# Farama-Foundation/Gymnasium-Robotics

Hardware: NVIDIA H100
Metric: env-steps/s (higher is better)
Workload: dtype f32

## Files before the change

### gymnasium_robotics_b200/csrc/b200sim.cu

```cuda
#include <cuda_runtime.h>
#include <stdio.h>
#include <stdlib.h>
#include <string>
#include <vector>

#include "../../include/b200sim.h"
#include "step_kernel.cuh"
#include "reset_sample.cuh"

#define B200_WPB_MAX 32

#ifdef B200_STAGE_TIMING
extern "C" int b200sim_debug_stage_cycles(unsigned long long* out, int reset) {
  cudaDeviceSynchronize();
  cudaMemcpyFromSymbol(out, g_stage_cycles, sizeof(unsigned long long) * TM_COUNT);
  if (reset) { unsigned long long z[TM_COUNT] = {0}; cudaMemcpyToSymbol(g_stage_cycles, z, sizeof(z)); }
  return TM_COUNT;
}
#endif

__global__ void reward_kernel(const float* __restrict__ ag, const float* __restrict__ dg, int M, int ngoal, int kind, float thr,
                              float radius, int dense, FetchTask task, float* __restrict__ out) {
  int i = blockIdx.x * blockDim.x + threadIdx.x;
  if (i >= M) return;
// ... 201 lines not shown
  if (t.kind == TASK_FETCH) { t.nact = 4; t.ngoal = 3; }
  if (t.kind == TASK_ADROIT_HAMMER) {
    bool ok = t.nact == dh->nu && t.ngoal == 3 && t.nobs == dh->nq - 6 + 6 + 13 && dh->nsensor <= 1 && t.penv_body > 0 && t.penv_body < dh->nb;
    const int sites[5] = {t.grip_site, t.obj_site, t.frame_site, t.tip_site[0], t.tip_site[1]};
    for (int k = 0; k < 5; k++) ok = ok && sites[k] >= 0 && sites[k] < dh->nsite;
    if (!ok) { delete h; return fail(nullptr, "b200sim_create: inconsistent AdroitHandHammer task", -6); }
  }
  if (t.kind == TASK_ADROIT_DOOR) {
    bool ok = t.nact == dh->nu && t.ngoal == 3 && t.nobs == dh->nq - 3 + 12 && t.penv_body > 0 && t.penv_body < dh->nb &&
              t.obj_qadr >= 0 && t.obj_qadr < dh->nq && t.grip_site >= 0 && t.grip_site < dh->nsite && t.frame_site >= 0 && t.frame_site < dh->nsite;
    if (!ok) { delete h; return fail(nullptr, "b200sim_create: inconsistent AdroitHandDoor task", -6); }
  }
  if (t.kind == TASK_ADROIT_PEN) {
    bool ok = t.nact == dh->nu && t.ngoal == 3 && t.nobs == dh->nq - 6 + 21 && t.penv_body > 0 && t.penv_body < dh->nb &&
              t.distance_threshold > 0 && t.rotation_threshold > 0;
    const int sites[6] = {t.obj_site, t.frame_site, t.tip_site[0], t.tip_site[1], t.tip_site[2], t.tip_site[3]};
    for (int k = 0; k < 6; k++) ok = ok && sites[k] >= 0 && sites[k] < dh->nsite;
    if (!ok) { delete h; return fail(nullptr, "b200sim_create: inconsistent AdroitHandPen task", -6); }
  }
  if (t.kind == TASK_ADROIT_RELOCATE) {
    bool ok = t.nact == dh->nu && t.ngoal == 3 && t.nobs == dh->nq - 6 + 9 && t.penv_body > 0 && t.penv_body < dh->nb &&
              t.grip_site >= 0 && t.grip_site < dh->nsite && t.obj_site >= 0 && t.obj_site < dh->nsite;
    if (!ok) { delete h; return fail(nullptr, "b200sim_create: inconsistent AdroitHandRelocate task", -6); }
  }
  if (t.kind == TASK_KITCHEN) {
    if (!(h->kitchen && t.nact == dh->nu && t.ngoal == dh->nq && t.nobs == dh->nq + dh->nv)) { delete h; return fail(nullptr, "b200sim_create: inconsistent FrankaKitchen task", -6); }
  } else if (h->kitchen) { delete h; return fail(nullptr, "b200sim_create: this model needs the kitchen task kind (8)", -6); }
  if (t.kind != TASK_FETCH && t.kind != TASK_ANTMAZE && t.kind != TASK_HAND && t.kind != TASK_HAND_REACH && !TASK_IS_ADROIT(t.kind) && t.kind != TASK_KITCHEN) { delete h; return fail(nullptr, "b200sim_create: unknown task kind", -6); }
  if (t.kind == TASK_HAND && (t.nact != dh->nu || t.ngoal != 7 || t.obj_qadr != dh->nq - 7 || t.obj_dadr != dh->nv - 6 ||
                              t.touch_mode < 0 || t.touch_mode > 3 || (t.touch_mode && dh->nsensor == 0) ||
                              t.nobs != t.obj_qadr + dh->nv + 7 + (t.touch_mode ? dh->nsensor : 0))) { delete h; return fail(nullptr, "b200sim_create: inconsistent Hand task", -6); }
  if (t.kind == TASK_FETCH && dh->nmocap != 1) { delete h; return fail(nullptr, "b200sim_create: Fetch task needs exactly one mocap body", -6); }
  if (t.kind == TASK_ANTMAZE && (t.nact != dh->nu || t.ngoal != 2 || t.touch_mode < 0 || t.touch_mode > 1 ||
                                 t.nobs != dh->nq - t.obs_qpos_start + dh->nv + (t.touch_mode == 1 ? 6 * (dh->nmjb - 1) : 0))) { delete h; return fail(nullptr, "b200sim_create: inconsistent AntMaze task", -6); }
  if (t.kind == TASK_HAND_REACH) {
    bool ok = t.nact == dh->nu && t.ngoal == 15 && t.nobs == dh->nq + dh->nv + 15;
    for (int k = 0; k < 5; k++) ok = ok && t.tip_site[k] >= 0 && t.tip_site[k] < dh->nsite;
    if (!ok) { delete h; return fail(nullptr, "b200sim_create: inconsistent HandReach task", -6); }
  }
  int o = 0;
  t.st_qpos = o; o += dh->nq; t.st_qvel = o; o += dh->nv; t.st_warm = o; o += dh->nv; t.st_ctrl = o; o += dh->nu;
  t.st_mocap = o; o += 7 * dh->nmocap; t.st_pose = o; o += (t.kind == TASK_FETCH ? 7 : 0); t.st_goal = o; o += t.ngoal;
  t.st_penv = o; o += (t.penv_body > 0 ? 7 : 0);
  t.st_stride = (o + 3) & ~3;
  DevGuard guard(device);
  if (!guard.ok) { delete h; return fail(nullptr, "b200sim_create: cudaSetDevice failed", -7); }
  int nsm = 132;
  cudaDeviceGetAttribute(&nsm, cudaDevAttrMultiProcessorCount, device);
  h->nvp = dh->nv <= 14 ? 14 : (dh->nv == 15 ? 15 : (dh->nv <= 21 ? 21 : (dh->nv <= 30 ? 30 : (dh->nv > 32 && dh->nv <= B200_WIDE_NVP ? B200_WIDE_NVP : 0))));
  if (h->nvp == 0) { delete h; return fail(nullptr, "b200sim_create: no kernel instantiation for this nv (31, 32 or > 36)", -8); }
  if ((t.kind == TASK_HAND || t.kind == TASK_HAND_REACH || TASK_IS_ADROIT(t.kind)) && h->nvp < 30) h->nvp = 30;
  if (dh->nv <= 21 && dh->any_convex_pair) h->nvp = 22;
  if (dh->nv <= 21 && (dh->nten > 0 || dh->nfric > 0 || dh->nsensor > 0 || dh->any_round_pair)) h->nvp = 30;
  auto fits = [&](int w) { return ((size_t)dh->hot_words + (size_t)w * dh->scr_words) * 4 + 64 <= 232448; };
  auto built = [&](int w) {
    if (h->nvp == B200_WIDE_NVP) return w == 7 || w == 10 || w == 13 || w == 14;
    bool b = false;
#define B200_HAS(W, V) b = b || (w == W && h->nvp == V);
    B200_FOR_ALL_VARIANTS(B200_HAS)
#undef B200_HAS
    return b;
  };
  const char* ov = getenv("B200SIM_WPB");
  const int ovw = ov ? atoi(ov) : 0;
  if (h->kitchen) {
    if (dh->nv > 31) { delete h; return fail(nullptr, "b200sim_create: the kitchen build is instantiated for nv <= 31", -8); }
    h->nvp = B200_KITCHEN_NVP;
    h->wpb = (num_envs + nsm - 1) / nsm <= 7 ? 7 : ((h->kitchen_groups && fits(11)) ? 11 : (fits(10) ? 10 : 7));
    if (ov) {
      if (!((ovw == 7 || ovw == 10 || (ovw == 11 && h->kitchen_groups)) && fits(ovw))) { delete h; return fail(nullptr, "b200sim_create: B200SIM_WPB names no kitchen kernel variant that fits", -8); }
      h->wpb = ovw;
    }
  } else {
    auto waves = [&](int w) { return ((num_envs + w - 1) / w + nsm - 1) / nsm; };
    int wmax = 0;
    for (int w = 1; w <= B200_WPB_MAX; w++)
      if (built(w) && fits(w)) wmax = w;
    h->wpb = wmax > 0 ? wmax : 7;
    for (int w = wmax; w >= 1; w--)
      if (built(w) && fits(w) && waves(w) == waves(wmax)) h->wpb = w;
    if (ov) {
      if (!(built(ovw) && fits(ovw))) { delete h; return fail(nullptr, "b200sim_create: B200SIM_WPB names no kernel variant that fits", -8); }
      h->wpb = ovw;
    }
  }
  if (!fits(h->wpb)) { delete h; return fail(nullptr, "b200sim_create: the per-env scratch of this model does not fit the shared memory of one block", -8); }
  h->smem_bytes = ((size_t)dh->hot_words + (size_t)h->wpb * dh->scr_words) * 4;
  h->blocks = (num_envs + h->wpb - 1) / h->wpb;
  h->packed_w = (t.nobs + 2 * t.ngoal + 4 + 3) & ~3;
  cudaError_t e = cudaErrorInvalidValue;
#define B200_SETATTR(W, V) if (h->wpb == W && h->nvp == V) e = cudaFuncSetAttribute(fetch_kernel<W, V>, cudaFuncAttributeMaxDynamicSharedMemorySize, (int)h->smem_bytes);
  B200_FOR_ALL_VARIANTS(B200_SETATTR)
#undef B200_SETATTR
  if (h->nvp == B200_WIDE_NVP) e = b200sim_wide_setattr(h->wpb, (int)h->smem_bytes) == 0 ? cudaSuccess : cudaErrorInvalidValue;
  if (h->nvp == B200_KITCHEN_NVP) e = (h->hull ? b200sim_kitchen_hull_setattr(h->wpb, (int)h->smem_bytes) : (h->kitchen_groups ? b200sim_kitchen_groups_setattr(h->wpb, (int)h->smem_bytes) : b200sim_kitchen_setattr(h->wpb, (int)h->smem_bytes))) == 0 ? cudaSuccess : cudaErrorInvalidValue;
  if (e != cudaSuccess) { std::string m = std::string("b200sim_create: no kernel variant <") + std::to_string(h->wpb) + ", " + std::to_string(h->nvp) + "> or cudaFuncSetAttribute(smem=" + std::to_string(h->smem_bytes) + ") failed: " + cudaGetErrorString(e); delete h; return fail(nullptr, m, -8); }
  const size_t state_bytes = (size_t)num_envs * t.st_stride * 4;
  if (cudaMalloc(&h->model_dev, h->model_host.size() * 4) != cudaSuccess || cudaMalloc(&h->state, state_bytes) != cudaSuccess ||
      cudaMalloc(&h->elapsed, (size_t)num_envs * 4) != cudaSuccess || cudaMalloc(&h->overflow_count, 8) != cudaSuccess) {
    free_handle(h); return fail(nullptr, "b200sim_create: cudaMalloc failed", -9);
  }
  if (cudaMemcpy(h->model_dev, h->model_host.data(), h->model_host.size() * 4, cudaMemcpyHostToDevice) != cudaSuccess ||
      cudaMemset(h->state, 0, state_bytes) != cudaSuccess || cudaMemset(h->elapsed, 0, (size_t)num_envs * 4) != cudaSuccess ||
      cudaMemset(h->overflow_count, 0, 8) != cudaSuccess) {
    free_handle(h); return fail(nullptr, "b200sim_create: uploading the model / clearing the state failed", -9);
  }
// ... 215 lines not shown
```

### gymnasium_robotics_b200/csrc/dmodel.h

```cpp
#pragma once
#include <stdint.h>
#include <string.h>
#include <math.h>
#include <vector>
#include <string>
#include <map>
#include <set>
#include <utility>

#include "../../include/b200sim_model.h"

#define DM_MAX_BODY 32
#define DM_MAX_NV 40
#define DM_NDOFROW_MIN 8
#define DM_NCAND_MAX 96
#define DM_NWELD_MAX 1
#define DM_CSLOT_WORDS 40

#ifdef B200_KITCHEN_GROUPS
#define DM_PAIR_HOT(X)
#define DM_PAIR_COLD(X) X(pair_geom1, 1, npair) X(pair_geom2, 1, npair) X(pair_margin, 1, npair)
#define DM_BGRP_HOT(X) X(bg_body, 1, nbgrp) X(bg_anchor, 1, nbgrp) X(bg_start, 1, nbgrp) X(bg_count, 1, nbgrp) X(bg_center, 3, nbgrp) X(bg_radius, 1, nbgrp)
#ifndef DM_NSURV_MAX
#define DM_NSURV_MAX 96
#endif
#else
#define DM_PAIR_HOT(X) X(pair_geom1, 1, npair) X(pair_geom2, 1, npair) X(pair_margin, 1, npair)
#define DM_PAIR_COLD(X)
#define DM_BGRP_HOT(X)
#endif
#ifdef B200_HULL
#define DM_HULL_COLD(X) X(geom_hull, 2, ngeom) X(hull_vert, 3, nhullv)
#else
#define DM_HULL_COLD(X)
#endif
#define DM_ARRAYS_HOT(X) \
  X(body_parent, 1, nb) X(body_jntadr, 1, nb) X(body_jntnum, 1, nb) X(body_dofadr, 1, nb) X(body_dofnum, 1, nb) \
  X(body_mocapid, 1, nb) X(body_ancdof, MW, nb) X(body_sub, 1, nb) X(body_pos, 3, nb) X(body_quat, 4, nb) \
  X(body_ipos, 3, nb) X(body_iquat, 4, nb) X(body_mass, 1, nb) X(body_inertia, 3, nb) \
  X(jnt_type, 1, njnt) X(jnt_body, 1, njnt) X(jnt_qposadr, 1, njnt) X(jnt_dofadr, 1, njnt) X(jnt_limited, 1, njnt) \
  X(jnt_pos, 3, njnt) X(jnt_axis, 3, njnt) X(jnt_range, 2, njnt) X(jnt_margin, 1, njnt) X(jnt_stiffness, 1, njnt) \
  X(jnt_qpos0, 1, njnt) X(jnt_qspring, 1, njnt) \
  X(dof_body, 1, nv) X(dof_jnt, 1, nv) X(dof_anc, MW, nv) X(dof_pre, MW, nv) X(dof_armature, 1, nv) \
  X(dof_damping, 1, nv) X(dof_frictionloss, 1, nv) X(dof_invweight0, 1, nv) \
  X(geom_type, 1, ngeom) X(geom_body, 1, ngeom) X(geom_pos, 3, ngeom) X(geom_quat, 4, ngeom) X(geom_size, 3, ngeom) \
  X(geom_rbound, 1, ngeom) \
  DM_PAIR_HOT(X) DM_BGRP_HOT(X) \
  X(site_body, 1, nsite) X(site_pos, 3, nsite) X(site_quat, 4, nsite) \
  X(act_trnid, 1, nu) X(act_ctrllimited, 1, nu) X(act_forcelimited, 1, nu) X(act_gear, 1, nu) X(act_gain, 1, nu) \
  X(act_bias, 3, nu) X(act_ctrlrange, 2, nu) X(act_forcerange, 2, nu) \
  X(eq_type, 1, neq) X(eq_obj1, 1, neq) X(eq_obj2, 1, neq) X(eq_active, 1, neq) X(eq_data, 11, neq) X(eq_solref, 2, neq) \
  X(eq_solimp, 5, neq) X(eq_invweight, 2, neq) \
  X(mocap_body, 1, nmocap) X(grid_walls, 1, ngridw) \
  X(dof_fricD, 1, nfric) X(dof_fricB, 1, nfric) \
  X(ten_dof, 2, nten) X(ten_qadr, 2, nten) X(ten_coef, 2, nten) X(ten_range, 2, nten) X(ten_margin, 1, nten)
#define DM_ARRAYS_COLD(X) \
  X(jnt_solref, 2, njnt) X(jnt_solimp, 5, njnt)  \
  DM_PAIR_COLD(X) \
  X(pair_condim, 1, npair) X(pair_friction, 3, npair) X(pair_gap, 1, npair) X(pair_solref, 2, npair) \
  X(pair_solimp, 5, npair) X(pair_invweight, 2, npair) \
  X(ten_solref, 2, nten) X(ten_solimp, 5, nten) X(ten_invweight, 1, nten) \
  X(sensor_site, 1, nsensor) X(sensor_body, 1, nsensor) X(sensor_type, 1, nsensor) X(sensor_size, 3, nsensor) \
  X(geom_mjb, 1, ngeom) X(mjb_rt, 1, nmjb)  \
  DM_HULL_COLD(X)
#define DM_ARRAYS(X) DM_ARRAYS_HOT(X) DM_ARRAYS_COLD(X)

#define DM_SCRATCH_PERSIST(X) \
  X(qpos, nq) X(qvel, nv) X(qacc, nv) X(ctrl, nu) X(mocap_pos, 3 * nmocap) X(mocap_quat, 4 * nmocap) \
  X(xpos, 3 * nb) X(xquat, 4 * nb) X(cdof, 6 * nv) X(M, nv * (nv + 1) / 2) X(fsmooth, nv) X(fcon, nv) \
  X(rk_q0, nrkq) X(rk_v0, nrkv) X(rk_dx, nrkv) X(rk_df, nrkv) \
// ... 3 lines not shown
#define DM_SCRATCH_UNION(X) X(kinA) X(kinB) X(cinert) X(b6) X(d6) X(geom_xpos) X(cand) X(surv) X(H) X(grad) X(search) X(Ma) X(Mv) X(cvel)
#else
#define DM_SCRATCH_UNION(X) X(kinA) X(kinB) X(cinert) X(b6) X(d6) X(geom_xpos) X(cand) X(H) X(grad) X(search) X(Ma) X(Mv) X(cvel)
#endif
#define DM_SCRATCH(X) DM_SCRATCH_PERSIST(X)

#ifdef B200_KITCHEN
enum { C_W = 0 , C_MU = 18 , C_D = 21, C_U = 22 , C_JV = 28 , C_DIMGRP = 34, CON_WORDS = 36 };
#define C_NB 6
#else
enum { C_W = 0 , C_MU = 18 , C_D = 20, C_U = 21 , C_JV = 25 , C_DIMGRP = 29, CON_WORDS = 30 };
#define C_NB 4
#endif
enum { FR_JAR = 0, FR_JV = 1 };
enum { CX_POS = 0, CX_PAIR = 3, CX_WORDS = 4 };
enum { DR_DOF = 0, DR_COEF = 1, DR_D = 2, DR_JAR = 3, DR_JV = 4, DR_DOF2 = 5, DR_COEF2 = 6, DR_WORDS = 7 };
enum { W_W = 0, W_D = 36, W_JAR = 42, W_JV = 48, W_B = 54, W_GRP = 55, WELD_WORDS = 56 };
#ifdef B200_WIDE
enum { G_RANGE = 0, G_MASK = 1, G_SIGN = 3, G_V = 5, GRP_WORDS = 11 };
#else
enum { G_RANGE = 0, G_MASK = 1, G_SIGN = 2, G_V = 3, GRP_WORDS = 9 };
#endif
enum { ROWT_EQ = 0, ROWT_FRICTION = 1, ROWT_LIMIT = 2 };
enum { CNT_NCON = 0, CNT_NDR = 1, CNT_NGRP = 2, CNT_NCAND = 3, CNT_NWELD = 4, CNT_ITERS = 5, CNT_OVERFLOW = 6 };

struct DMHead {
  int nb, njnt, nq, nv, nu, ngeom, nsite, nmocap, neq, npair;
  int nwords;
  int hot_words;
  int scr_words;
  int iterations, ls_iterations, integrator, any_damping, kin_iters, ncon_max, ngrp_max, ndr_max;
  int edges_per_con, any_convex_pair, mask_words, penv_body;
  int nten, nfric, ncand_max, nsensor;
  int grid_len, grid_wid, ngridw, any_round_pair;
  int nmjb;
  int s_cslotA, ncslotA, s_cslotB, ncslotB;
  float grid_scale, grid_top, grid_xc, grid_yc;
  float timestep, gravity[3], tolerance, impratio, meaninertia, ls_tolerance, ref[3];
#define X(name, w, kind) int o_##name;
  DM_ARRAYS(X)
#undef X
#define X(name, words) int s_##name;
  DM_SCRATCH_PERSIST(X)
#undef X
#define X(name) int s_##name;
  DM_SCRATCH_UNION(X)
#undef X
#ifdef B200_KITCHEN_GROUPS
  int nbgrp;
#endif
};

static inline uint32_t f2w(float f) { uint32_t u; memcpy(&u, &f, 4); return u; }

static inline int dm_build(const b200_model_view& m, const double* eq_data_override, const float ref[3],
                           std::vector<uint32_t>& buf, std::string& err, int penv_body = -1, bool force_wide = false,
                           int ngrp_cap = 0 ) {
  DMHead h;
  memset(&h, 0, sizeof(h));
  h.nb = m.nbody; h.njnt = m.njnt; h.nq = m.nq; h.nv = m.nv; h.nu = m.nu; h.nsite = m.nsite;
  h.nmocap = m.nmocap; h.neq = m.neq;
  std::vector<int> psrc;
  std::vector<int> pgrid;
  {
    std::vector<char> seen(m.ngeom, 0);
    for (int p = 0; p < m.npair; p++) {
      bool isgrid = m.n_pair_grid == m.npair && m.pair_grid[p];
      if (!isgrid) { psrc.push_back(p); pgrid.push_back(0); }
      else if (!seen[m.pair_geom1[p]]) { seen[m.pair_geom1[p]] = 1; psrc.push_back(p); pgrid.push_back(1); }
    }
  }
#ifdef B200_KITCHEN_GROUPS
  struct BGroup { int body, anchor, start, count; double c[3], r; };
  std::vector<BGroup> bgs;
  {
    std::map<std::pair<int, int>, std::vector<int>> buckets;
    for (size_t p = 0; p < psrc.size(); p++) {
      if (pgrid[p]) { err = "maze-grid pairs are not part of the kitchen build"; return -1; }
      buckets[std::make_pair(m.geom_body[m.pair_geom1[psrc[p]]], m.geom_body[m.pair_geom2[psrc[p]]])].push_back(psrc[p]);
    }
    std::vector<int> order;
    for (auto& kv : buckets) {
      const std::vector<int>& ps = kv.second;
      std::set<int> GA, GB;
      for (int sp : ps) { GA.insert(m.pair_geom1[sp]); GB.insert(m.pair_geom2[sp]); }
      int ba = kv.first.first, bb = kv.first.second;
      bool anchorB = ba == 0 ? false : (bb == 0 ? true : GB.size() <= GA.size());
      const std::set<int>& anchors = anchorB ? GB : GA;
      for (int an : anchors) {
        BGroup g;
        g.body = anchorB ? ba : bb; g.anchor = an; g.start = (int)order.size(); g.count = 0;
        std::vector<int> partner;
        double mg = 0;
        for (int sp : ps) {
          if ((anchorB ? m.pair_geom2[sp] : m.pair_geom1[sp]) != an) continue;
          order.push_back(sp); g.count++;
          partner.push_back(anchorB ? m.pair_geom1[sp] : m.pair_geom2[sp]);
          if (m.pair_margin[sp] > mg) mg = m.pair_margin[sp];
        }
        for (int k = 0; k < 3; k++) { g.c[k] = 0; for (int pg : partner) g.c[k] += m.geom_pos[3 * pg + k] / partner.size(); }
        g.r = 0;
        for (int pg : partner) {
          double d2 = 0;
          for (int k = 0; k < 3; k++) { double d = m.geom_pos[3 * pg + k] - g.c[k]; d2 += d * d; }
          double rr = sqrt(d2) + m.geom_rbound[pg];
          if (rr > g.r) g.r = rr;
// ... 219 lines not shown
      F(h.o_geom_size, 3 * g + 0, 2 * (q[1] * q[3] + q[0] * q[2])); F(h.o_geom_size, 3 * g + 1, 2 * (q[2] * q[3] - q[0] * q[1]));
      F(h.o_geom_size, 3 * g + 2, q[0] * q[0] - q[1] * q[1] - q[2] * q[2] + q[3] * q[3]);
    }
    for (int k = 0; k < 4; k++) F(h.o_geom_quat, 4 * g + k, m.geom_quat[4 * sg + k]);
    F(h.o_geom_rbound, g, m.geom_rbound[sg]);
    I(h.o_geom_mjb, g, m.n_geom_mjbody == m.ngeom ? m.geom_mjbody[sg] : m.geom_body[sg]);
#ifdef B200_HULL
    I(h.o_geom_hull, 2 * g, m.geom_hull[2 * sg]); I(h.o_geom_hull, 2 * g + 1, m.geom_hull[2 * sg + 1]);
    if (m.geom_type[sg] == B200_GEOM_MESH && m.geom_hull[2 * sg + 1] < 4) { err = "mesh geom without a hull vertex table"; return -1; }
#else
    if (m.geom_type[sg] == B200_GEOM_MESH) { err = "mesh geoms need the hull build of the library (models compiled without mesh_hull carry box proxies)"; return -1; }
#endif
  }
#ifdef B200_HULL
  for (int i = 0; i < 3 * nhullv; i++) F(h.o_hull_vert, i, m.hull_vert[i]);
#endif
  for (int p = 0; p < npair; p++) {
    int sp = psrc[p];
    I(h.o_pair_geom1, p, gmap[m.pair_geom1[sp]]); I(h.o_pair_geom2, p, pgrid[p] ? -1 : gmap[m.pair_geom2[sp]]); I(h.o_pair_condim, p, m.pair_condim[sp]);
    int t1 = m.geom_type[m.pair_geom1[sp]], t2 = m.geom_type[m.pair_geom2[sp]];
    bool r1 = t1 == B200_GEOM_SPHERE || t1 == B200_GEOM_CAPSULE, r2 = t2 == B200_GEOM_SPHERE || t2 == B200_GEOM_CAPSULE;
    bool c1 = t1 == B200_GEOM_CYLINDER || t1 == B200_GEOM_ELLIPSOID, c2 = t2 == B200_GEOM_CYLINDER || t2 == B200_GEOM_ELLIPSOID;
    bool v1 = r1 || c1 || t1 == B200_GEOM_BOX, v2 = r2 || c2 || t2 == B200_GEOM_BOX;
    bool ok = (t1 == B200_GEOM_PLANE && (t2 == B200_GEOM_BOX || r2 || c2)) || (t1 == B200_GEOM_BOX && t2 == B200_GEOM_BOX) ||
              (r1 && t2 == B200_GEOM_BOX) || (r1 && r2) || ((c1 || c2) && v1 && v2);
#ifdef B200_HULL
    {
      bool m1 = t1 == B200_GEOM_MESH, m2 = t2 == B200_GEOM_MESH;
      if ((t1 == B200_GEOM_PLANE && m2) || ((m1 || m2) && (v1 || m1) && (v2 || m2))) { ok = true; c1 = c1 || m1; c2 = c2 || m2; }
    }
#endif
    if (r1 && r2) h.any_round_pair = 1;
    if (c1 || c2) h.any_convex_pair = 1;

    if (!ok) { err = "collision pair type not supported by the CUDA path yet"; return -1; }
#ifdef B200_KITCHEN
    if (m.pair_condim[sp] != 1 && m.pair_condim[sp] != 3 && m.pair_condim[sp] != 4 && m.pair_condim[sp] != 6) { err = "condim must be 1, 3, 4 or 6"; return -1; }
#else
    if (m.pair_condim[sp] != 1 && m.pair_condim[sp] != 3 && m.pair_condim[sp] != 4) { err = "condim must be 1, 3 or 4 on the CUDA path"; return -1; }
#endif
    F(h.o_pair_friction, 3 * p + 0, m.pair_friction[5 * sp + 0]); F(h.o_pair_friction, 3 * p + 1, m.pair_friction[5 * sp + 2]);
    F(h.o_pair_friction, 3 * p + 2, m.pair_friction[5 * sp + 3]);
    F(h.o_pair_margin, p, m.pair_margin[sp]); F(h.o_pair_gap, p, m.pair_gap[sp]);
    for (int k = 0; k < 2; k++) { F(h.o_pair_solref, 2 * p + k, m.pair_solref[2 * sp + k]); F(h.o_pair_invweight, 2 * p + k, m.pair_invweight[2 * sp + k]); }
    for (int k = 0; k < 5; k++) F(h.o_pair_solimp, 5 * p + k, m.pair_solimp[5 * sp + k]);
  }
#ifdef B200_KITCHEN_GROUPS
  for (int g = 0; g < nbgrp; g++) {
    I(h.o_bg_body, g, bgs[g].body); I(h.o_bg_anchor, g, gmap[bgs[g].anchor]); I(h.o_bg_start, g, bgs[g].start); I(h.o_bg_count, g, bgs[g].count);
    for (int k = 0; k < 3; k++) F(h.o_bg_center, 3 * g + k, bgs[g].c[k]);
    F(h.o_bg_radius, g, bgs[g].r);
  }
#endif
  if (3 * (h.edges_per_con * ncon_max + 6 * DM_NWELD_MAX + ndr_max) > h.s_grad - h.s_H) { err = "line-search edge list does not fit the solver scratch"; return -1; }
  for (int k = 0; k < nsensor; k++) {
    I(h.o_sensor_site, k, m.sensor_site[k]); I(h.o_sensor_body, k, m.sensor_body[k]); I(h.o_sensor_type, k, m.sensor_type[k]);
    for (int a = 0; a < 3; a++) F(h.o_sensor_size, 3 * k + a, m.sensor_size[3 * k + a]);
  }
  for (int i = 0; i < h.grid_len * h.grid_wid; i++) if (m.grid_walls[i]) buf[h.o_grid_walls + i / 32] |= 1u << (i % 32);
  for (int s = 0; s < nsite; s++) {
    I(h.o_site_body, s, m.site_body[s]);
    for (int k = 0; k < 3; k++) F(h.o_site_pos, 3 * s + k, m.site_pos[3 * s + k]);
    for (int k = 0; k < 4; k++) F(h.o_site_quat, 4 * s + k, m.site_quat[4 * s + k]);
  }
  for (int a = 0; a < nu; a++) {
    I(h.o_act_trnid, a, m.act_trnid[a]); I(h.o_act_ctrllimited, a, m.act_ctrllimited[a]); I(h.o_act_forcelimited, a, m.act_forcelimited[a]);
    F(h.o_act_gear, a, m.act_gear[a]); F(h.o_act_gain, a, m.act_gainprm[3 * a]);
    for (int k = 0; k < 3; k++) F(h.o_act_bias, 3 * a + k, m.act_biasprm[3 * a + k]);
    for (int k = 0; k < 2; k++) { F(h.o_act_ctrlrange, 2 * a + k, m.act_ctrlrange[2 * a + k]); F(h.o_act_forcerange, 2 * a + k, m.act_forcerange[2 * a + k]); }
  }
  for (int e = 0; e < neq; e++) {
#ifdef B200_KITCHEN
    if (m.eq_type[e] != B200_EQ_WELD && m.eq_type[e] != B200_EQ_JOINT) { err = "only weld and joint equalities are supported"; return -1; }
#else
    if (m.eq_type[e] != B200_EQ_WELD) { err = "only weld equalities are supported by the CUDA path yet"; return -1; }
#endif
    I(h.o_eq_type, e, m.eq_type[e]); I(h.o_eq_obj1, e, m.eq_obj1[e]); I(h.o_eq_obj2, e, m.eq_obj2[e]); I(h.o_eq_active, e, m.eq_active[e]);
    const double* data = eq_data_override ? eq_data_override + 11 * e : m.eq_data + 11 * e;
    for (int k = 0; k < 11; k++) F(h.o_eq_data, 11 * e + k, data[k]);
    for (int k = 0; k < 2; k++) { F(h.o_eq_solref, 2 * e + k, m.eq_solref[2 * e + k]); F(h.o_eq_invweight, 2 * e + k, m.eq_invweight[2 * e + k]); }
    for (int k = 0; k < 5; k++) F(h.o_eq_solimp, 5 * e + k, m.eq_solimp[5 * e + k]);
  }
  for (int i = 0; i < nmocap; i++) I(h.o_mocap_body, i, m.mocap_body[i]);
  for (int b = 0; b < nmjb; b++) I(h.o_mjb_rt, b, m.n_mjbody_rt > 0 ? m.mjbody_rt[b] : b);
  if (nmjb > 255) { err = "more than 255 MJCF bodies"; return -1; }
  memcpy(buf.data(), &h, sizeof(h));
  return 0;
}
```

### gymnasium_robotics_b200/csrc/sim_core.cuh

```cuda
#pragma once
#include "dmodel.h"

#if defined(__CUDACC__) || defined(B200_HOST_WARP)
#define B200_WARP_CODE 1
#endif
#ifdef __CUDACC__
#define HD static __device__ __forceinline__
#define HDN static __device__ __noinline__
#define STAGE static __device__ __noinline__
#define ASSUME_SHARED_PTR(p) __builtin_assume(__isShared(p))
#define ASSUME_SHARED(c) do { __builtin_assume(__isShared((c).s)); __builtin_assume(__isShared((c).mw)); __builtin_assume(__isShared((c).h)); } while (0)
#define WARP_W 32
#define SYNC() __syncwarp()
#ifdef B200_BLOCK_ALIGN
#ifdef B200_ALIGN_SYNCWARP
#define ALIGN() do { __syncwarp(); __syncthreads(); } while (0)
#define ALIGN_OR(p) (__syncwarp(), __syncthreads_or(p))
#elif defined(B200_AG)
static __device__ __forceinline__ void b200_bar_g(int id, int nthreads) { asm volatile("bar.sync %0, %1;" ::"r"(id), "r"(nthreads) : "memory"); }
static __device__ __forceinline__ bool b200_bar_or_g(int id, int nthreads, bool p) {
  int r;
  asm volatile("{ .reg .pred q, r; setp.ne.s32 q, %3, 0; bar.red.or.pred r, %1, %2, q; selp.s32 %0, 1, 0, r; }" : "=r"(r) : "r"(id), "r"(nthreads), "r"((int)p) : "memory");
  return r != 0;
}
// ... 1973 lines not shown
    for (int r = k + 1; r < KB; r++) S[r][k] *= inv;
#pragma unroll
    for (int r = k + 1; r < KB; r++)
#pragma unroll
      for (int q = k + 1; q <= r; q++) S[r][q] = fmaf(-S[r][k], S[q][k], S[r][q]);
  }
#pragma unroll
  for (int k = 0; k < NA; k++) {
    float yk = __shfl_sync(FULL, b * dinv, k);
    float bn = fmaf(-h[k], yk, b);
    b = (i > k) ? bn : ((i == k) ? yk : b);
  }
#pragma unroll
  for (int r = 0; r < KB; r++) bb[r] -= wsum(cb[r] * b);
#pragma unroll
  for (int k = 0; k < KB; k++) {
    bb[k] *= sinv[k];
#pragma unroll
    for (int r = k + 1; r < KB; r++) bb[r] = fmaf(-S[r][k], bb[k], bb[r]);
  }
#pragma unroll
  for (int k = KB - 1; k >= 0; k--) {
    bb[k] *= sinv[k];
#pragma unroll
    for (int r = 0; r < k; r++) bb[r] = fmaf(-S[k][r], bb[k], bb[r]);
  }
#pragma unroll
  for (int r = 0; r < KB; r++) b = fmaf(-cb[r], bb[r], b);
  float sacc = 0.f, z = 0.f;
#pragma unroll
  for (int k = NA - 1; k >= 0; k--) {
    float zk = __shfl_sync(FULL, (b - dinv * sacc) * dinv, k);
    float sn = fmaf(h[k], zk, sacc);
    sacc = (i < k) ? sn : sacc;
    z = (i == k) ? zk : z;
  }
  __syncwarp();
  if (i < nv && i < NA) x[i] = z;
#pragma unroll
  for (int r = 0; r < KB; r++) if (i == r && 32 + r < nv) x[32 + r] = bb[r];
  __syncwarp();
}
#else
template <int NVP>
static inline void spd_solve(const Ctx& c, const float* A, const float* dadd, float hh, float* x, float* scratchH) {
  int nv = c.h->nv, nM = nv * (nv + 1) / 2;
  for (int i = 0; i < nM; i++) scratchH[i] = A[i];
  if (dadd) for (int i = 0; i < nv; i++) scratchH[i * (i + 1) / 2 + i] += hh * dadd[i];
  cholesky(c, scratchH);
  chol_solve(c, scratchH, x);
}
#endif

template <bool HF>
STAGE int ls_edges(const Ctx c) {
  ASSUME_SHARED(c);
  const DMHead* h = c.h;
  const int* cnt = SI(counters);
  const int epc = h->edges_per_con, ncon = cnt[CNT_NCON], nweld6 = cnt[CNT_NWELD] * 6, ndr = cnt[CNT_NDR];
  float* E = SF(H);
  LANES(i, ncon) {
    const float* cr = SF(con) + i * CON_WORDS;
    float* e = E + 3 * epc * i;
    int dim = con_dim(cr);
    float D = cr[C_D], un = cr[C_U], vn = cr[C_JV];
    int ne = 0;
    if (dim == 1) { e[0] = un; e[1] = vn; e[2] = D; ne = 1; }
    else for (int k = 1; k < dim; k++) {
      float mu = con_mu(cr, k), uk = mu * cr[C_U + k], vk = mu * cr[C_JV + k];
      e[3 * ne] = un + uk; e[3 * ne + 1] = vn + vk; e[3 * ne + 2] = D; ne++;
      e[3 * ne] = un - uk; e[3 * ne + 1] = vn - vk; e[3 * ne + 2] = D; ne++;
    }
    for (; ne < epc; ne++) e[3 * ne + 2] = 0.f;
  }
  float* W = E + 3 * epc * ncon;
  LANES(i, nweld6) {
    const float* wr = SF(weld) + (i / 6) * WELD_WORDS;
    int k = i % 6;
    W[3 * i] = wr[W_JAR + k]; W[3 * i + 1] = wr[W_JV + k]; W[3 * i + 2] = -wr[W_D + k];
  }
  float* R = W + 3 * nweld6;
  LANES(i, ndr) {
    const float* dr = SF(dofrow) + i * DR_WORDS;
    R[3 * i] = dr[DR_JAR]; R[3 * i + 1] = dr[DR_JV]; R[3 * i + 2] = dr[DR_D];
  }
  SYNC();
  return epc * ncon + nweld6 + ndr;
}

template <bool HF>
STAGE void ls_eval(const Ctx c, int nedge, float alpha, float g1, float g2, float* out) {
  ASSUME_SHARED(c);
  float cost = 0, d1 = 0, d2 = 0;
  const float* E = SF(H);
  LANES(i, nedge) {
    float x0 = E[3 * i], v = E[3 * i + 1], D = E[3 * i + 2];
    float x = fmaf(alpha, v, x0), Da = fabsf(D);
    if (D < 0 || (x < 0 && D > 0)) { float dx = Da * x; cost = fmaf(0.5f * dx, x, cost); d1 = fmaf(dx, v, d1); d2 = fmaf(Da * v, v, d2); }
  }
  if (HF) LANES(d, c.h->nfric) {
    float D = MF(dof_fricD)[d];
    if (D > 0) {
      float fl = MF(dof_frictionloss)[d], v = SF(fric)[c.h->nfric + d], x = SF(fric)[d] + alpha * v, Rf = fl / D;
      if (x <= -Rf) { cost += fl * (-0.5f * Rf - x); d1 -= fl * v; }
      else if (x >= Rf) { cost += fl * (-0.5f * Rf + x); d1 += fl * v; }
      else { cost += 0.5f * D * x * x; d1 += D * x * v; d2 += D * v * v; }
    }
  }
  out[0] = wsum(cost) + alpha * g1 + alpha * alpha * g2;
  out[1] = wsum(d1) + g1 + 2 * alpha * g2;
  out[2] = wsum(d2) + 2 * g2;
}

template <bool HF>
STAGE float linesearch(const Ctx c, float g1, float g2, float gtol, int maxit, float* improve) {
  ASSUME_SHARED(c);
  float p0[3], p[3];
  const int nedge = ls_edges<HF>(c);
  ls_eval<HF>(c, nedge, 0.f, g1, g2, p0);
  *improve = 0;
  if (p0[1] >= 0 || p0[2] <= 0) return 0.f;
  gtol = fmaxf(gtol, 1e-5f * fabsf(p0[1]));
  float lo = 0, hi = -1, alpha = -p0[1] / p0[2], best = 0, bestcost = p0[0];
  for (int it = 0; it < maxit; it++) {
    ls_eval<HF>(c, nedge, alpha, g1, g2, p);
    if (p[0] <= bestcost) { bestcost = p[0]; best = alpha; }
    if (fabsf(p[1]) < gtol) break;
    if (p[1] < 0) lo = alpha; else hi = alpha;
    float next = alpha - p[1] / p[2];
    if (hi > 0 && (next <= lo || next >= hi)) next = 0.5f * (lo + hi);
    if (next == alpha) break;
    alpha = next;
  }
  *improve = p0[0] - bestcost;
  return best;
}

template <bool HF>
STAGE void newton_begin(const Ctx c) {
  ASSUME_SHARED(c);
  mulM(c, SF(qacc), SF(Ma));
  rows_begin<HF>(c, SF(qvel), SF(qacc));
}

template <bool HF>
STAGE int newton_check(const Ctx c, int iter, float improvement) {
  ASSUME_SHARED(c);
  const DMHead* h = c.h;
  int nv = h->nv;
  float *Ma = SF(Ma), *grad = SF(grad), *fs = SF(fsmooth), *fcon = SF(fcon);
  float scale = 1.0f / (h->meaninertia * (float)(nv > 1 ? nv : 1));
  float tol = fmaxf(h->tolerance, 1e-6f);
  TIC();
  pass_F<HF>(c, fcon);
  TOC(TM_CK_PASSF);
  float g2sum = 0, f2sum = 0;
  LANES(i, nv) {
    float g = Ma[i] - fs[i] - fcon[i], f = fabsf(Ma[i]) + fabsf(fs[i]) + fabsf(fcon[i]);
    grad[i] = g; g2sum += g * g; f2sum += f * f;
  }
  SYNC();
  float gnorm = sqrtf(wsum(g2sum)), fnorm = sqrtf(wsum(f2sum));
#if defined(B200_DEBUG_SOLVER) && !defined(__CUDACC__)
  printf("  iter %d gnorm %.3e fnorm %.3e improvement %.3e\n", iter, gnorm, fnorm, improvement);
#endif
  if (gnorm < 2e-6f * fnorm) return 1;
  if (iter > 0 && (scale * improvement < tol || scale * gnorm < tol)) return 1;
  if (iter >= h->iterations || iter >= 12) return 1;
  return 0;
}

template <int NVP>
STAGE void newton_direction(const Ctx c) {
  ASSUME_SHARED(c);
  int nv = c.h->nv;
  LANES(i, nv) SF(search)[i] = -SF(grad)[i];
  SYNC();
  spd_solve<NVP>(c, SF(H), nullptr, 0.f, SF(search), SF(H));
}

template <bool HF>
STAGE int newton_move(const Ctx c, float* improvement) {
  ASSUME_SHARED(c);
  const DMHead* h = c.h;
  int nv = h->nv;
  int* cnt = SI(counters);
  float *a = SF(qacc), *Ma = SF(Ma), *Mv = SF(Mv), *search = SF(search), *fs = SF(fsmooth);
  float scale = 1.0f / (h->meaninertia * (float)(nv > 1 ? nv : 1));
  TIC();
  mulM(c, search, Mv);
  TOC(TM_MV_MULM);
  rows_from_vec<HF>(c, search);
  TOC(TM_MV_ROWS);
  float q1 = 0, q2 = 0, sn = 0;
  LANES(i, nv) { q1 += search[i] * (Ma[i] - fs[i]); q2 += 0.5f * search[i] * Mv[i]; sn += search[i] * search[i]; }
  q1 = wsum(q1); q2 = wsum(q2); sn = sqrtf(wsum(sn));
  if (sn < 1e-20f) return 1;
  float gtol = h->tolerance * h->ls_tolerance * sn / scale;
  TOC(TM_MV_ROWS);
  float alpha = linesearch<HF>(c, q1, q2, gtol, h->ls_iterations < 20 ? h->ls_iterations : 20, improvement);
  TOC(TM_MV_LS);
  if (alpha == 0.f) return 1;
  LANES(i, nv) { a[i] += alpha * search[i]; Ma[i] += alpha * Mv[i]; }
  LANES(i, cnt[CNT_NCON]) { float* cr = SF(con) + i * CON_WORDS; for (int k = 0; k < C_NB; k++) cr[C_U + k] += alpha * cr[C_JV + k]; }
  LANES(i, cnt[CNT_NWELD] * 6) { float* wr = SF(weld) + (i / 6) * WELD_WORDS; wr[W_JAR + i % 6] += alpha * wr[W_JV + i % 6]; }
  LANES(i, cnt[CNT_NDR]) { float* dr = SF(dofrow) + i * DR_WORDS; dr[DR_JAR] += alpha * dr[DR_JV]; }
  if (HF) LANES(d, h->nfric) SF(fric)[d] += alpha * SF(fric)[h->nfric + d];
  SYNC();
  if (c.lane == 0) cnt[CNT_ITERS] += 1;
  TOC(TM_MV_UPD);
  return 0;
}

template <int NVP>
STAGE void euler_solve(const Ctx c) {
  ASSUME_SHARED(c);
  const DMHead* h = c.h;
  float* x = SF(search);
  LANES(i, h->nv) x[i] = SF(fsmooth)[i] + SF(fcon)[i];
  SYNC();
  spd_solve<NVP>(c, SF(M), MF(dof_damping), h->timestep, x, SF(H));
}

#ifndef B200_ALIGN_LEVEL
#define B200_ALIGN_LEVEL 3
#endif
#define ALIGN_LEVEL_FOR(NVP) ((NVP) >= 30 ? 4 : B200_ALIGN_LEVEL)
#define ALIGN_AT(level) do { if (kAlign >= (level)) ALIGN(); } while (0)
template <int NVP, bool REBUILD = false>
HD void forward(const Ctx c, bool active, bool* euler_solved = nullptr) {
  constexpr bool HF = NVP >= 30;
  constexpr bool CX = NVP == 22 || NVP >= 30;
  constexpr int kAlign = ALIGN_LEVEL_FOR(NVP);
  TIC();
#ifndef B200_NO_ALIGN_FIRST
  ALIGN_AT(1); TOC(TM_BARRIER);
#endif
  if (active) kinematics(stage_ctx<REBUILD>(c));
  TOC(TM_KIN); ALIGN_AT(4); TOC(TM_BARRIER);
  if (active) { com_quantities(stage_ctx<REBUILD>(c)); mass_matrix(stage_ctx<REBUILD>(c)); }
#ifndef B200_NO_ALIGN_PRECOLL
  TOC(TM_COM_M); ALIGN_AT(2); TOC(TM_BARRIER);
#endif
  if (active) collision<HF, CX>(stage_ctx<REBUILD>(c));
  TOC(TM_COLL); ALIGN_AT(2); TOC(TM_BARRIER);
  if (active) make_constraint<HF>(stage_ctx<REBUILD>(c));
  TOC(TM_CONSTR); ALIGN_AT(4); TOC(TM_BARRIER);
  if (active) smooth_forces(stage_ctx<REBUILD>(c));
  TOC(TM_SMOOTH); ALIGN_AT(4); TOC(TM_BARRIER);
  if (active) newton_begin<HF>(stage_ctx<REBUILD>(c));
  TOC(TM_NBEGIN);
  int done = active ? 0 : 1;
  float improvement = 0;
  if (kAlign >= 3) {
    for (int iter = 0;; iter++) {
      ALIGN(); TOC(TM_BARRIER);
      if (!done) done = newton_check<HF>(stage_ctx<REBUILD>(c), iter, improvement);
      TOC(TM_NCHECK);
      bool more = ALIGN_OR(!done);
      TOC(TM_BARRIER);
      if (!more) break;
      if (!done) build_H<HF>(stage_ctx<REBUILD>(c));
      TOC(TM_BUILDH); ALIGN_AT(4); TOC(TM_BARRIER);
      if (!done) newton_direction<NVP>(stage_ctx<REBUILD>(c));
#ifdef B200_EULER_PIGGYBACK
      else if (euler_solved && active && !*euler_solved && c.h->any_damping) { euler_solve<NVP>(stage_ctx<REBUILD>(c)); *euler_solved = true; }
#endif
      TOC(TM_NDIR); ALIGN(); TOC(TM_BARRIER);
      if (!done) done = newton_move<HF>(stage_ctx<REBUILD>(c), &improvement) ? 2 : 0;
      TOC(TM_NMOVE);
    }
  } else {
    ALIGN_AT(2);
    for (int iter = 0; !done; iter++) {
      done = newton_check<HF>(c, iter, improvement);
      if (done) break;
      build_H<HF>(c);
      newton_direction<NVP>(c);
      done = newton_move<HF>(c, &improvement) ? 2 : 0;
    }
  }
}

STAGE void integrate_pos(const Ctx c, float* qpos, const float* qvel, float hh) {
  ASSUME_SHARED(c);
  ASSUME_SHARED_PTR(qpos); ASSUME_SHARED_PTR(qvel);
  const DMHead* h = c.h;
  LANES(j, h->njnt) {
    int a = MI(jnt_qposadr)[j], d = MI(jnt_dofadr)[j];
    if (MI(jnt_type)[j] == B200_JNT_FREE) {
      for (int k = 0; k < 3; k++) qpos[a + k] += hh * qvel[d + k];
      float w[3] = {qvel[d + 3], qvel[d + 4], qvel[d + 5]};
      float n = sqrtf(dot3(w, w));
      float q[4] = {qpos[a + 3], qpos[a + 4], qpos[a + 5], qpos[a + 6]};
      if (n > 0) {
        float ang = 0.5f * n * hh, sn = sinf(ang), cs = cosf(ang), inv = 1.0f / n;
        float dq[4] = {cs, w[0] * inv * sn, w[1] * inv * sn, w[2] * inv * sn}, nq[4];
        qmul(nq, q, dq);
        q[0] = nq[0]; q[1] = nq[1]; q[2] = nq[2]; q[3] = nq[3];
      }
      qnormalize(q);
      qpos[a + 3] = q[0]; qpos[a + 4] = q[1]; qpos[a + 5] = q[2]; qpos[a + 6] = q[3];
    } else qpos[a] += hh * qvel[d];
  }
  SYNC();
}

template <int NVP>
STAGE void euler_step(const Ctx c, bool solved = false) {
  ASSUME_SHARED(c);
  const DMHead* h = c.h;
  int nv = h->nv;
  float hh = h->timestep;
  float* x = SF(search);
  if (h->any_damping) {
    if (!solved) euler_solve<NVP>(c);
  } else {
    LANES(i, nv) x[i] = SF(qacc)[i];
    SYNC();
  }
  LANES(i, nv) SF(qvel)[i] += hh * x[i];
  SYNC();
  integrate_pos(c, SF(qpos), SF(qvel), hh);
}

template <int NVP, bool REBUILD = false>
HD void rk4_substep(const Ctx c, bool active) {
  const DMHead* h = c.h;
  const int nv = h->nv, nq = h->nq;
  const float hh = h->timestep;
  const float A[3] = {0.5f, 0.5f, 1.0f}, B[4] = {1.0f / 6, 1.0f / 3, 1.0f / 3, 1.0f / 6};
  if (active) {
// ... 27 lines not shown
```

Baseline: 1.050 million.

## Keep line-search constraint edges in registers instead of shared scratch

For non-kitchen builds, the Newton line search now builds each lane's constraint edges (position, velocity, D) once into per-thread register arrays sized by a compile-time edges-per-lane bound, and re-evaluates cost and derivatives from registers on every iteration. The old path wrote an edge list to shared scratch and re-read it on each evaluation. This aims to cut shared-memory traffic and syncs inside the line-search loop. In exchange it raises register pressure and adds a host-side check that rejects models needing more edges than the register budget.

```diff
diff --git a/gymnasium_robotics_b200/csrc/b200sim.cu b/gymnasium_robotics_b200/csrc/b200sim.cu
--- a/gymnasium_robotics_b200/csrc/b200sim.cu
+++ b/gymnasium_robotics_b200/csrc/b200sim.cu
@@ -277,6 +277,11 @@
   if ((t.kind == TASK_HAND || t.kind == TASK_HAND_REACH || TASK_IS_ADROIT(t.kind)) && h->nvp < 30) h->nvp = 30;
   if (dh->nv <= 21 && dh->any_convex_pair) h->nvp = 22;
   if (dh->nv <= 21 && (dh->nten > 0 || dh->nfric > 0 || dh->nsensor > 0 || dh->any_round_pair)) h->nvp = 30;
+  if (!h->kitchen && dm_ls_edges(*dh) > 32 * DM_LS_E(h->nvp)) {
+    std::string m = "b200sim_create: the line search of the NVP = " + std::to_string(h->nvp) + " kernel build holds " + std::to_string(32 * DM_LS_E(h->nvp)) +
+                    " constraint edges per env, this model needs up to " + std::to_string(dm_ls_edges(*dh));
+    delete h; return fail(nullptr, m, -8);
+  }
   auto fits = [&](int w) { return ((size_t)dh->hot_words + (size_t)w * dh->scr_words) * 4 + 64 <= 232448; };
   auto built = [&](int w) {
     if (h->nvp == B200_WIDE_NVP) return w == 7 || w == 10 || w == 13 || w == 14;
diff --git a/gymnasium_robotics_b200/csrc/dmodel.h b/gymnasium_robotics_b200/csrc/dmodel.h
--- a/gymnasium_robotics_b200/csrc/dmodel.h
+++ b/gymnasium_robotics_b200/csrc/dmodel.h
@@ -16,6 +16,11 @@
 #define DM_NCAND_MAX 96
 #define DM_NWELD_MAX 1
 #define DM_CSLOT_WORDS 40
+#ifdef B200_KITCHEN
+#define DM_LS_E(NVP) 0
+#else
+#define DM_LS_E(NVP) ((NVP) >= 30 ? 6 : 5)
+#endif
 
 #ifdef B200_KITCHEN_GROUPS
 #define DM_PAIR_HOT(X)
@@ -125,6 +130,7 @@
 };
 
 static inline uint32_t f2w(float f) { uint32_t u; memcpy(&u, &f, 4); return u; }
+static inline int dm_ls_edges(const DMHead& h) { return h.edges_per_con * h.ncon_max + 6 * DM_NWELD_MAX + h.ndr_max; }
 
 static inline int dm_build(const b200_model_view& m, const double* eq_data_override, const float ref[3],
                            std::vector<uint32_t>& buf, std::string& err, int penv_body = -1, bool force_wide = false,
@@ -450,7 +456,9 @@
     F(h.o_bg_radius, g, bgs[g].r);
   }
 #endif
-  if (3 * (h.edges_per_con * ncon_max + 6 * DM_NWELD_MAX + ndr_max) > h.s_grad - h.s_H) { err = "line-search edge list does not fit the solver scratch"; return -1; }
+#ifdef B200_KITCHEN
+  if (3 * dm_ls_edges(h) > h.s_grad - h.s_H) { err = "line-search edge list does not fit the solver scratch"; return -1; }
+#endif
   for (int k = 0; k < nsensor; k++) {
     I(h.o_sensor_site, k, m.sensor_site[k]); I(h.o_sensor_body, k, m.sensor_body[k]); I(h.o_sensor_type, k, m.sensor_type[k]);
     for (int a = 0; a < 3; a++) F(h.o_sensor_size, 3 * k + a, m.sensor_size[3 * k + a]);
diff --git a/gymnasium_robotics_b200/csrc/sim_core.cuh b/gymnasium_robotics_b200/csrc/sim_core.cuh
--- a/gymnasium_robotics_b200/csrc/sim_core.cuh
+++ b/gymnasium_robotics_b200/csrc/sim_core.cuh
@@ -2049,6 +2049,103 @@
 }
 #endif
 
+struct LsStep { float alpha, improve; };
+#ifndef B200_KITCHEN
+struct LsVal { float cost, d1, d2; };
+
+HD float pyramid_edge(float xn, float mu, float xk) {
+#ifdef __CUDACC__
+  return fmaf(mu, xk, xn);
+#else
+  return xn + mu * xk;
+#endif
+}
+
+template <bool HF, int NS>
+HD LsVal ls_eval(const Ctx c, const float (&ex)[NS], const float (&ev)[NS], const float (&eD)[NS], int nedge, float alpha, float g1,
+                 float g2) {
+  float cost = 0, d1 = 0, d2 = 0;
+#pragma unroll
+  for (int j = 0; j < NS; j++) {
+    if (WARP_W * j >= nedge) break;
+    float x0 = ex[j], v = ev[j], D = eD[j];
+    float x = fmaf(alpha, v, x0), Da = fabsf(D);
+    if (D < 0 || (x < 0 && D > 0)) { float dx = Da * x; cost = fmaf(0.5f * dx, x, cost); d1 = fmaf(dx, v, d1); d2 = fmaf(Da * v, v, d2); }
+  }
+  if (HF) LANES(d, c.h->nfric) {
+    float D = MF(dof_fricD)[d];
+    if (D > 0) {
+      float fl = MF(dof_frictionloss)[d], v = SF(fric)[c.h->nfric + d], x = SF(fric)[d] + alpha * v, Rf = fl / D;
+      if (x <= -Rf) { cost += fl * (-0.5f * Rf - x); d1 -= fl * v; }
+      else if (x >= Rf) { cost += fl * (-0.5f * Rf + x); d1 += fl * v; }
+      else { cost += 0.5f * D * x * x; d1 += D * x * v; d2 += D * v * v; }
+    }
+  }
+  LsVal r;
+  r.cost = wsum(cost) + alpha * g1 + alpha * alpha * g2;
+  r.d1 = wsum(d1) + g1 + 2 * alpha * g2;
+  r.d2 = wsum(d2) + 2 * g2;
+  return r;
+}
+
+template <bool HF, int LSE>
+HD LsStep linesearch(const Ctx c, float g1, float g2, float gtol, int maxit) {
+  ASSUME_SHARED(c);
+  constexpr int NS = LSE * 32 / WARP_W;
+  const DMHead* h = c.h;
+  const int* cnt = SI(counters);
+  const int epc = h->edges_per_con, ncon = cnt[CNT_NCON], nweld6 = cnt[CNT_NWELD] * 6, ndr = cnt[CNT_NDR];
+  const int nce = epc * ncon, nwe = nce + nweld6, nedge = nwe + ndr;
+  float ex[NS], ev[NS], eD[NS];
+  const int qs = WARP_W / epc, rs = WARP_W % epc;
+  int q = c.lane / epc, r = c.lane % epc;
+#pragma unroll
+  for (int j = 0; j < NS; j++) {
+    const int e = c.lane + WARP_W * j;
+    float x0 = 0.f, v = 0.f, D = 0.f;
+    if (j > 0) { q += qs; r += rs; if (r >= epc) { r -= epc; q++; } }
+    if (WARP_W * j < nedge) {
+      if (e < nce) {
+        const float* cr = SF(con) + q * CON_WORDS;
+        const int k = r, dim = con_dim(cr);
+        const float un = cr[C_U], vn = cr[C_JV];
+        if (dim == 1) {
+          if (k == 0) { x0 = un; v = vn; D = cr[C_D]; }
+        } else if (k < 2 * (dim - 1)) {
+          const int b = 1 + (k >> 1);
+          const float mu = con_mu(cr, b), su = (k & 1) ? -cr[C_U + b] : cr[C_U + b], sv = (k & 1) ? -cr[C_JV + b] : cr[C_JV + b];
+          x0 = pyramid_edge(un, mu, su); v = pyramid_edge(vn, mu, sv);
+          D = cr[C_D];
+        }
+      } else if (e < nwe) {
+        const int i = e - nce;
+        const float* wr = SF(weld) + (i / 6) * WELD_WORDS;
+        x0 = wr[W_JAR + i % 6]; v = wr[W_JV + i % 6]; D = -wr[W_D + i % 6];
+      } else if (e < nedge) {
+        const float* dr = SF(dofrow) + (e - nwe) * DR_WORDS;
+        x0 = dr[DR_JAR]; v = dr[DR_JV]; D = dr[DR_D];
+      }
+    }
+    ex[j] = x0; ev[j] = v; eD[j] = D;
+  }
+  const LsVal p0 = ls_eval<HF>(c, ex, ev, eD, nedge, 0.f, g1, g2);
+  if (p0.d1 >= 0 || p0.d2 <= 0) return LsStep{0.f, 0.f};
+  gtol = fmaxf(gtol, 1e-5f * fabsf(p0.d1));
+  float lo = 0, hi = -1, alpha = -p0.d1 / p0.d2, best = 0, bestcost = p0.cost;
+  for (int it = 0; it < maxit; it++) {
+    const LsVal p = ls_eval<HF>(c, ex, ev, eD, nedge, alpha, g1, g2);
+    if (p.cost <= bestcost) { bestcost = p.cost; best = alpha; }
+    if (fabsf(p.d1) < gtol) break;
+    if (p.d1 < 0) lo = alpha; else hi = alpha;
+    float next = alpha - p.d1 / p.d2;
+    if (hi > 0 && (next <= lo || next >= hi)) next = 0.5f * (lo + hi);
+    if (next == alpha) break;
+    alpha = next;
+  }
+  return LsStep{best, p0.cost - bestcost};
+}
+
+#else
 template <bool HF>
 STAGE int ls_edges(const Ctx c) {
   ASSUME_SHARED(c);
@@ -2109,14 +2206,13 @@
   out[2] = wsum(d2) + 2 * g2;
 }
 
-template <bool HF>
-STAGE float linesearch(const Ctx c, float g1, float g2, float gtol, int maxit, float* improve) {
+template <bool HF, int LSE>
+STAGE LsStep linesearch(const Ctx c, float g1, float g2, float gtol, int maxit) {
   ASSUME_SHARED(c);
   float p0[3], p[3];
   const int nedge = ls_edges<HF>(c);
   ls_eval<HF>(c, nedge, 0.f, g1, g2, p0);
-  *improve = 0;
-  if (p0[1] >= 0 || p0[2] <= 0) return 0.f;
+  if (p0[1] >= 0 || p0[2] <= 0) return LsStep{0.f, 0.f};
   gtol = fmaxf(gtol, 1e-5f * fabsf(p0[1]));
   float lo = 0, hi = -1, alpha = -p0[1] / p0[2], best = 0, bestcost = p0[0];
   for (int it = 0; it < maxit; it++) {
@@ -2129,9 +2225,10 @@
     if (next == alpha) break;
     alpha = next;
   }
-  *improve = p0[0] - bestcost;
-  return best;
-}
+  return LsStep{best, p0[0] - bestcost};
+}
+
+#endif
 
 template <bool HF>
 STAGE void newton_begin(const Ctx c) {
@@ -2176,7 +2273,7 @@
   spd_solve<NVP>(c, SF(H), nullptr, 0.f, SF(search), SF(H));
 }
 
-template <bool HF>
+template <bool HF, int LSE>
 STAGE int newton_move(const Ctx c, float* improvement) {
   ASSUME_SHARED(c);
   const DMHead* h = c.h;
@@ -2195,7 +2292,9 @@
   if (sn < 1e-20f) return 1;
   float gtol = h->tolerance * h->ls_tolerance * sn / scale;
   TOC(TM_MV_ROWS);
-  float alpha = linesearch<HF>(c, q1, q2, gtol, h->ls_iterations < 20 ? h->ls_iterations : 20, improvement);
+  const LsStep ls = linesearch<HF, LSE>(c, q1, q2, gtol, h->ls_iterations < 20 ? h->ls_iterations : 20);
+  *improvement = ls.improve;
+  const float alpha = ls.alpha;
   TOC(TM_MV_LS);
   if (alpha == 0.f) return 1;
   LANES(i, nv) { a[i] += alpha * search[i]; Ma[i] += alpha * Mv[i]; }
@@ -2229,6 +2328,7 @@
   constexpr bool HF = NVP >= 30;
   constexpr bool CX = NVP == 22 || NVP >= 30;
   constexpr int kAlign = ALIGN_LEVEL_FOR(NVP);
+  constexpr int kLsE = DM_LS_E(NVP);
   TIC();
 #ifndef B200_NO_ALIGN_FIRST
   ALIGN_AT(1); TOC(TM_BARRIER);
@@ -2264,7 +2364,7 @@
       else if (euler_solved && active && !*euler_solved && c.h->any_damping) { euler_solve<NVP>(stage_ctx<REBUILD>(c)); *euler_solved = true; }
 #endif
       TOC(TM_NDIR); ALIGN(); TOC(TM_BARRIER);
-      if (!done) done = newton_move<HF>(stage_ctx<REBUILD>(c), &improvement) ? 2 : 0;
+      if (!done) done = newton_move<HF, kLsE>(stage_ctx<REBUILD>(c), &improvement) ? 2 : 0;
       TOC(TM_NMOVE);
     }
   } else {
@@ -2274,7 +2374,7 @@
       if (done) break;
       build_H<HF>(c);
       newton_direction<NVP>(c);
-      done = newton_move<HF>(c, &improvement) ? 2 : 0;
+      done = newton_move<HF, kLsE>(c, &improvement) ? 2 : 0;
     }
   }
 }
```

New measurement: 1.095 million (median of 6 runs). 1.04x the previous value.
